# mickeyjoe666/PHFPFAC

Hardware: AMD Instinct MI355X
Metric: input GB/s scanned (higher is better)
Workload: dtype u8

## Files before the change

### phfpfac_amd/csrc/pfac_hip.hip

```cpp
#include <hip/hip_runtime.h>
#include <hip/hip_ext.h>

#include <stdint.h>
#include <stdio.h>
#include <stdlib.h>
#include <string.h>

#include <algorithm>
#include <chrono>
#include <mutex>
#include <type_traits>
#include <string>
#include <vector>

#include "pfac.h"
#include "pfac_fold.h"

namespace {

constexpr int WAVE = 64;
constexpr int SUB = WAVE * 16;
constexpr int SUBS = 4;
constexpr int WTILE = SUB * SUBS;
constexpr int MSUBS = 2;
// ... 749 lines not shown
    auto log_put = [&](bool f, unsigned word) {
        const unsigned long long b = __builtin_amdgcn_ballot_w64(f);
        if (b) {
            if (f) stg[(lc + lane_rank(b)) & (STG - 1u)] = word;
            lc += (unsigned)__popcll(b);
        }
    };
    auto log_flush = [&](bool all) {
        if (lc - fl >= (unsigned)WAVE || (all && lc != fl)) {
            wave_lds_sync();
            while (lc - fl >= (unsigned)WAVE) {
                __builtin_amdgcn_raw_buffer_store_b32(stg[(fl + (unsigned)lane) & (STG - 1u)], lrs, (int)((fl + (unsigned)lane) << 2), 0, 0);
                fl += WAVE;
            }
            if (all && fl + (unsigned)lane < lc)
                __builtin_amdgcn_raw_buffer_store_b32(stg[(fl + (unsigned)lane) & (STG - 1u)], lrs, (int)((fl + (unsigned)lane) << 2), 0, 0);
        }
    };
    auto slot = [&](int i) -> int4 {
        return *reinterpret_cast<const int4 *>(reinterpret_cast<const unsigned char *>(a.T4) + ((unsigned)i << 4));
    };
    auto slot_of = [&](int rnv, unsigned st, unsigned byte) -> int {
        return W8 ? rnv + (int)byte : rnv + (int)(((st & ((1u << sub) - 1u)) << 8) | byte);
    };
    const bool edge = own_end < (unsigned)WTILE || lim < (unsigned)WTILE + 3u;
    const unsigned n2 = (unsigned)a.d1_n2;
    auto front = [&](auto edge_c) {
        constexpr bool EDGE = decltype(edge_c)::value;
        unsigned p[D2_FB], win[D2_FB], rt[D2_FB], col[D2_FB];
        int nx[D2_FB];
        int2 e2[D2_FB];
#pragma unroll
        for (int u = 0; u < D2_FB; u++) {
            p[u] = P0 + (unsigned)(u * WAVE + lane);
            const unsigned lo = t32[p[u] >> 2], hi = t32[(p[u] >> 2) + 1];
            win[u] = __builtin_amdgcn_alignbyte(hi, lo, p[u] & 3u);
        }
#pragma unroll
        for (int u = 0; u < D2_FB; u++) {
            rt[u] = t0[win[u] & 0xFFu];
            col[u] = d1.colmap[(win[u] >> 8) & 0xFFu];
        }
#pragma unroll
        for (int u = 0; u < D2_FB; u++) {
            if (EDGE && p[u] >= own_end) rt[u] = no_root;
            nx[u] = d1.rows[(rt[u] >> 16) + col[u]];
        }
#pragma unroll
        for (int u = 0; u < D2_FB; u++) {
            if (EDGE && p[u] + 1u >= lim) nx[u] = -1;
            const unsigned ri = (unsigned)(nx[u] >> D1_STATE_BITS);
            e2[u] = d1.r2[ri < n2 ? ri : n2];
        }
#pragma unroll
        for (int u = 0; u < D2_FB; u++) {
            const unsigned s1 = rt[u] & 0xFFFFu, s2 = (unsigned)nx[u] & ((1u << D1_STATE_BITS) - 1u);
            const bool fin1 = s1 != 0xFFFFu, fin2 = s2 < nfin;
            const unsigned b2 = (win[u] >> 16) & 0xFFu;
#ifdef PFAC_ABL_D2NOWALK
            const bool more = false && b2;
#else
            const bool more = (((unsigned)e2[u].y >> (b2 & 31u)) & 1u) != 0u && (!EDGE || p[u] + 2u < lim);
#endif
            log_put(fin1, p[u] | (s1 << 16));
            log_put(fin2, p[u] | (fin1 ? 1u << 12 : 0u) | ((unsigned)nx[u] << 16));
            const unsigned long long mb = __builtin_amdgcn_ballot_w64(more);
            if (mb) {
                const unsigned n12 = (fin1 ? 1u : 0u) + (fin2 ? 1u : 0u);
                if (more) ring[(head + fcount + lane_rank(mb)) & (unsigned)(D2_RING - 1)] =
                    make_uint2(p[u] | ((unsigned)nx[u] << 12), (unsigned)slot_of(e2[u].x, s2, b2) | (n12 << 28));
                fcount += (unsigned)__popcll(mb);
            }
        }
        P0 += D2_FB * WAVE;
    };
#ifdef PFAC_TRACE_BUILD
    unsigned long long tq_front = 0, tq_iter = 0, tq_n = 0;
    const unsigned long long tq_t0 = __builtin_amdgcn_s_memrealtime();
#endif
    for (;;) {
        unsigned long long dm[NS];
        unsigned nd = 0;
#pragma unroll
        for (int w = 0; w < NS; w++) { dm[w] = __builtin_amdgcn_ballot_w64(!alive[w]); nd += (unsigned)__popcll(dm[w]); }
#ifdef PFAC_TRACE_BUILD
        const unsigned long long tq_a = __builtin_amdgcn_s_memrealtime();
#endif
        while (fcount < nd && P0 < own_end && fcount <= (unsigned)(D2_RING - D2_FB * WAVE)) {
            if (edge) front(std::true_type{}); else front(std::false_type{});
            log_flush(false);
        }
#ifdef PFAC_TRACE_BUILD
        tq_front += __builtin_amdgcn_s_memrealtime() - tq_a;
        tq_n++;
#endif
        if (nd == (unsigned)(NS * WAVE) && fcount == 0u) break;
        wave_lds_sync();
#pragma unroll
        for (int w = 0; w < NS; w++) {
            if (fcount && dm[w]) {
                const unsigned free_n = (unsigned)__popcll(dm[w]);
                const unsigned take = free_n < fcount ? free_n : fcount;
                const unsigned rk = lane_rank(dm[w]);
                if (!alive[w] && rk < take) {
                    const uint2 e = ring[(head + rk) & (unsigned)(D2_RING - 1)];
                    pos[w] = e.x & 0xFFFu;
                    s[w] = (int)(e.x >> 12);
                    idx[w] = (int)(e.y & 0x0FFFFFFFu);
                    jn[w] = e.y >> 28;
                    pn[w] = pos[w] + 2u;
                    alive[w] = true;
                }
                head += take;
                fcount -= take;
            }
        }
        int4 e4[NS];
        unsigned nb[NS];
#pragma unroll
        for (int w = 0; w < NS; w++) {
            e4[w] = make_int4(-1, -1, 0, 0);
            if (alive[w]) e4[w] = slot(idx[w]);
        }
#pragma unroll
        for (int w = 0; w < NS; w++) nb[w] = tile[alive[w] ? pn[w] + 1u : 0u];
#pragma unroll
        for (int w = 0; w < NS; w++) {
            const bool ok = alive[w] && e4[w].x == (W8 ? s[w] : (s[w] >> sub));
            const int sn = e4[w].y;
            const bool fin = ok && (unsigned)sn < nfin;
            log_put(fin, pos[w] | ((jn[w] & 15u) << 12) | ((unsigned)sn << 16));
            jn[w] += fin ? 1u : 0u;
            jmax |= jn[w];
            pn[w] += 1u;
            alive[w] = ok && pn[w] < lim && (((unsigned)e4[w].w >> (nb[w] & 31u)) & 1u) != 0u;
            s[w] = sn;
            idx[w] = slot_of(e4[w].z, (unsigned)sn, nb[w]);
        }
        log_flush(false);
    }
    log_flush(true);
#ifdef PFAC_TRACE_BUILD
    if (a.dbg && blockIdx.x < 8 && lane == 0 && (threadIdx.x >> 6) == 0) {
        unsigned long long *acc = a.dbg + (size_t)blockIdx.x * 64 * 32 + 10;
        const unsigned long long tq_all = __builtin_amdgcn_s_memrealtime() - tq_t0;
        acc[0] += tq_front; acc[1] += tq_n; acc[2] += tq_all; acc[3] += 1; acc[4] += lc;
    }
    (void)tq_iter;
#endif
    if (__any(jmax > 15u) || lc > logcap) return ~0u;
    return lc;
}

__device__ __forceinline__ void dense2_scatter(const ScanArgs &a, unsigned char *aux, const unsigned *logg, unsigned cnt,
                                               unsigned long long base, int lane) {
    unsigned *cntw = reinterpret_cast<unsigned *>(aux + D2_CNT_OFF);
    unsigned *pref2 = reinterpret_cast<unsigned *>(aux + D2_PREF_OFF);
    const unsigned short *pref = reinterpret_cast<const unsigned short *>(aux + D2_PREF_OFF);
    auto nibsum = [](unsigned x) -> unsigned { return (((x & 0x0F0F0F0Fu) + ((x >> 4) & 0x0F0F0F0Fu)) * 0x01010101u) >> 24; };
    constexpr int UN = 4;
    constexpr int ER = 32;
    const u32x4 zero4 = {0u, 0u, 0u, 0u};
    reinterpret_cast<u32x4 *>(cntw)[lane] = zero4;
    reinterpret_cast<u32x4 *>(cntw)[lane + WAVE] = zero4;
    wave_lds_sync();
    const unsigned long long room = base < a.out_cap ? a.out_cap - base : 0ull;
    const __amdgpu_buffer_rsrc_t ors = __builtin_amdgcn_make_buffer_rsrc(static_cast<unsigned *>(a.out) + base, 0,
                                                                         (int)((room < (unsigned long long)cnt ? (unsigned)room : cnt) * 4u), 0x00020000);
    auto count_one = [&](unsigned e) { atomicAdd(&cntw[(e & 0xFFFu) >> 3], 1u << ((e & 7u) * 4u)); };
    auto prefix = [&]() {
        wave_lds_sync();
        const u32x4 x0 = reinterpret_cast<const u32x4 *>(cntw)[2 * lane], x1 = reinterpret_cast<const u32x4 *>(cntw)[2 * lane + 1];
        unsigned sm[8];
#pragma unroll
        for (int k = 0; k < 4; k++) { sm[k] = nibsum(x0[k]); sm[4 + k] = nibsum(x1[k]); }
        unsigned tot = 0;
#pragma unroll
        for (int k = 0; k < 8; k++) tot += sm[k];
        unsigned run = wave_incl_scan(tot) - tot;
        u32x4 pw;
#pragma unroll
        for (int k = 0; k < 4; k++) {
            const unsigned lo = run; run += sm[2 * k];
            const unsigned hi = run; run += sm[2 * k + 1];
            pw[k] = lo | (hi << 16);
        }
        reinterpret_cast<u32x4 *>(pref2)[lane] = pw;
        wave_lds_sync();
    };
    auto place_one = [&](unsigned e) {
        const unsigned p = e & 0xFFFu, j = (e >> 12) & 15u, st = e >> 16;
        const unsigned x = cntw[p >> 3];
        const unsigned dest = (unsigned)pref[p >> 3] + nibsum(x & ((1u << ((p & 7u) * 4u)) - 1u)) + j;
        __builtin_amdgcn_raw_buffer_store_b32(p | (st << 12), ors, (int)(dest << 2), 0, 0);
    };
    if (cnt <= (unsigned)(ER * WAVE)) {
        const __amdgpu_buffer_rsrc_t lrs = __builtin_amdgcn_make_buffer_rsrc(const_cast<unsigned *>(logg), 0, (int)(cnt * 4u), 0x00020000);
        unsigned e[ER];
#pragma unroll
        for (int g = 0; g < ER / UN; g++) {
            if ((unsigned)(g * UN * WAVE) < cnt) {
#pragma unroll
                for (int u = 0; u < UN; u++)
                    e[g * UN + u] = __builtin_amdgcn_raw_buffer_load_b32(lrs, lane * 4, (g * UN + u) * WAVE * 4, 0);
            }
        }
#pragma unroll
        for (int g = 0; g < ER / UN; g++) {
            if ((unsigned)(g * UN * WAVE) < cnt) {
#pragma unroll
                for (int u = 0; u < UN; u++)
                    if ((unsigned)((g * UN + u) * WAVE + lane) < cnt) count_one(e[g * UN + u]);
            }
        }
        prefix();
#ifdef PFAC_ABL_D2NOSCATTER
        cnt = 0;
#endif
#pragma unroll
        for (int g = 0; g < ER / UN; g++) {
            if ((unsigned)(g * UN * WAVE) < cnt) {
#pragma unroll
                for (int u = 0; u < UN; u++)
                    if ((unsigned)((g * UN + u) * WAVE + lane) < cnt) place_one(e[g * UN + u]);
            }
        }
        return;
    }
    for (unsigned i0 = 0; i0 < cnt; i0 += UN * WAVE) {
        unsigned e[UN];
#pragma unroll
        for (int u = 0; u < UN; u++) {
            const unsigned i = i0 + (unsigned)(u * WAVE + lane);
            e[u] = i < cnt ? logg[i] : 0u;
        }
#pragma unroll
        for (int u = 0; u < UN; u++)
            if (i0 + (unsigned)(u * WAVE + lane) < cnt) count_one(e[u]);
    }
    prefix();
#ifdef PFAC_ABL_D2NOSCATTER
    cnt = 0;
#endif
    for (unsigned i0 = 0; i0 < cnt; i0 += UN * WAVE) {
        unsigned e[UN];
#pragma unroll
        for (int u = 0; u < UN; u++) {
            const unsigned i = i0 + (unsigned)(u * WAVE + lane);
            e[u] = i < cnt ? logg[i] : 0u;
        }
#pragma unroll
        for (int u = 0; u < UN; u++)
            if (i0 + (unsigned)(u * WAVE + lane) < cnt) place_one(e[u]);
    }
}

template <int ROOT>
__device__ __forceinline__ unsigned root_mask(const u32x4 w, const unsigned char *ftab, unsigned root_x4) {
    if (ROOT == 1) {
        unsigned nm[4];
#pragma unroll
        for (int i = 0; i < 4; i++) {
            const unsigned x = w[i] ^ root_x4;
            nm[i] = (((x & 0x7F7F7F7Fu) + 0x7F7F7F7Fu) | x) & 0x80808080u;
        }
        unsigned lo = __builtin_amdgcn_udot4(nm[0], 0x08040201u, 0u, false);
        lo = __builtin_amdgcn_udot4(nm[1], 0x80402010u, lo, false);
        unsigned hi = __builtin_amdgcn_udot4(nm[2], 0x08040201u, 0u, false);
        hi = __builtin_amdgcn_udot4(nm[3], 0x80402010u, hi, false);
        return ~((lo >> 7) | (hi << 1)) & 0xFFFFu;
    } else {
        const unsigned char *t8 = ftab;
        unsigned p = 0;
#pragma unroll
        for (int g = 0; g < 4; g++) {
            const unsigned d = w[g];
            const unsigned v = (unsigned)t8[d & 0xFFu] | (unsigned)t8[256 + ((d >> 8) & 0xFFu)] |
                               (unsigned)t8[512 + ((d >> 16) & 0xFFu)] | (unsigned)t8[768 + (d >> 24)];
            p |= v << (8 * g);
        }
        unsigned x = p & 0x0F0F0F0Fu, y = (p >> 4) & 0x0F0F0F0Fu;
        x = (x | (x >> 4)) & 0x00FF00FFu; y = (y | (y >> 4)) & 0x00FF00FFu;
        x = (x | (x >> 8)) & 0xFFFFu; y = (y | (y >> 8)) & 0xFFFFu;
        return x | (y << 16);
    }
}

__device__ __forceinline__ unsigned eq_mask32(const u32x4 lo16, const u32x4 hi16, unsigned x4) {
    return root_mask<1>(lo16, nullptr, x4) | (root_mask<1>(hi16, nullptr, x4) << 16);
}

#ifdef PFAC_TRACE_BUILD
#define PFAC_STAMP(cond, slot) do { if (cond) tr[slot] = __builtin_amdgcn_s_memrealtime(); } while (0)
#else
#define PFAC_STAMP(cond, slot) do { } while (0)
#endif

#ifndef PFAC_SPARSE_FUSED_NW
#define PFAC_SPARSE_FUSED_NW 2
#endif
constexpr int MAX_WAVES_NW4 = 10;

template <bool TLDS, bool W8, int ROOT, bool FUSED, int NW, int NB, bool FOLD>
__device__ __forceinline__ void scan_body(const ScanArgs &a, unsigned char *smem, const ErrCh &err) {
    unsigned *hdr = reinterpret_cast<unsigned *>(smem + SH_HDR);
    int *s0 = reinterpret_cast<int *>(smem + SH_S0);
    unsigned char *ftab = smem + SH_FTAB;
    unsigned char *finl = smem + SH_FIN;
    const int tid = threadIdx.x;
    const int lane = tid & (WAVE - 1);
    const int wave = __builtin_amdgcn_readfirstlane(tid >> 6);
    const int nc = (int)(blockDim.x >> 6) - 1;

    for (unsigned i = blockIdx.x * blockDim.x + tid; i < a.zero_vec; i += gridDim.x * blockDim.x)
        a.zero_next[i] = make_uint4(0u, 0u, 0u, 0u);
    for (int i = tid; i < H_WORDS; i += blockDim.x) hdr[i] = 0;
    for (int i = tid; i < 256; i += blockDim.x) {
        const int v = a.s0[i];
        const bool sec2 = a.sec2[i] != 0;
        s0[i] = v;
        finl[i] = (unsigned)v < (unsigned)a.num_final ? (unsigned char)1 : (unsigned char)0;
#pragma unroll
        for (int k = 0; k < 4; k++)
            ftab[k * 256 + i] = (unsigned char)((v >= 0 ? 1u << k : 0u) | (sec2 ? 1u << (k + 4) : 0u));
    }
    unsigned char *d1idx_l = smem + SH_D1IDX;
    int *d1_l = reinterpret_cast<int *>(smem + SH_D1);
    unsigned char *colmap_l = smem + SH_COLMAP;
    if (a.d1_rows > 0) {
        for (int i = tid; i < 256; i += blockDim.x) { d1idx_l[i] = a.d1idx[i]; colmap_l[i] = a.d1_colmap[i]; }
        for (int i = tid; i < a.d1_rows * a.d1_stride; i += blockDim.x) {
            const int row = i / a.d1_stride, c = i - row * a.d1_stride;
            d1_l[i] = c < a.d1_ncols ? a.d1[row * 256 + a.d1_colbyte[c]] : -1;
        }
    } else {
        for (int i = tid; i < 256; i += blockDim.x) { d1idx_l[i] = 0; colmap_l[i] = 0; }
    }
    if (a.d1_rows > 0)
        for (int i = tid; i < a.d1_stride; i += blockDim.x) d1_l[a.d1_rows * a.d1_stride + i] = -1;
    const unsigned *t0_l = reinterpret_cast<const unsigned *>(smem + a.sh_t0);
    if (FUSED && NW == 4 && a.sh_t0)
        for (int i = tid; i < 256; i += blockDim.x) {
            const int v = a.s0[i];
            reinterpret_cast<unsigned *>(smem + a.sh_t0)[i] = v >= 0 ? (((unsigned)v < (unsigned)a.num_final ? (unsigned)v : 0xFFFFu) | ((unsigned)(a.d1idx[i] * a.d1_stride) << 16))
                                                                     : (0xFFFFu | ((unsigned)(a.d1_rows * a.d1_stride) << 16));
        }
    int2 *d1r2_l = reinterpret_cast<int2 *>(smem + SH_D1 + a.d1_lds_bytes);
    if (FUSED && a.d1_n2 > 0)
        for (int i = tid; i <= a.d1_n2; i += blockDim.x) {
            const int2 e = i < a.d1_n2 ? a.d1r2[i] : make_int2(-a.rn_bias, 0);
            d1r2_l[i] = make_int2(e.x + a.rn_bias, e.y);
        }
    int *s0r_l = reinterpret_cast<int *>(smem + SH_D1);
    const bool have_s0r = FUSED && a.d1_rows == 0;
    if (have_s0r)
        for (int i = tid; i < 256; i += blockDim.x) {
            const int v = a.s0[i];
            s0r_l[i] = v >= 0 ? a.r[v >> (a.wbit - 8)] + a.rn_bias : 0;
        }
    const Dense1 d1 = {colmap_l, d1idx_l, d1_l, a.d1_rows > 0, (FUSED && a.d1_n2 > 0) ? d1r2_l : nullptr, have_s0r ? s0r_l : nullptr};
    const int sh_tab = SH_D1 + a.d1_lds_bytes;
    const int *R = a.r;
    const int2 *T = a.T;
    if (TLDS) {
        int *lr = reinterpret_cast<int *>(smem + sh_tab);
        int2 *lt = reinterpret_cast<int2 *>(smem + sh_tab + ((a.r_words * 4 + 15) & ~15));
        for (int i = tid; i < a.r_words; i += blockDim.x) lr[i] = a.r[i];
        for (int i = tid; i < a.t_entries; i += blockDim.x) lt[i] = a.T[i];
        R = lr;
        T = lt;
    }
    const unsigned char *bm2l = smem + a.sh_bm2;
    if (a.l2f_mode == 2) {
        const unsigned *src = reinterpret_cast<const unsigned *>(a.bm2 + (ROOT == 1 ? (a.root_byte & 0xFFu) * 32u : 0u));
        unsigned *dst = reinterpret_cast<unsigned *>(smem + a.sh_bm2);
        for (int i = tid; i < a.bm2_rows * 8; i += blockDim.x) dst[i] = src[i];
    }
    __syncthreads();
#ifdef PFAC_TRACE_BUILD
    if (a.dbg && blockIdx.x < 8 && threadIdx.x == 0) a.dbg[((size_t)blockIdx.x * 64 + 1) * 32 + 15] = __builtin_amdgcn_s_memrealtime();
#endif

#ifdef PFAC_ABL_NOCOORD
    if (wave == nc) return;
#endif
    if (wave == nc) {
        __builtin_amdgcn_s_setprio(3);
#ifdef PFAC_ABL_STATIC
        unsigned abl_seq = 0;
        auto ticket = [&]() -> unsigned { return (abl_seq++) * gridDim.x + blockIdx.x; };
#else
        auto ticket = [&]() -> unsigned {
            unsigned g = 0;
            if (lane == 0) g = atomicAdd(&a.ctl[(blockIdx.x % a.ticket_ways) * 64u], 1u) * a.ticket_ways + blockIdx.x % a.ticket_ways;
            return g;
        };
#endif
        auto publish_batch = [&](unsigned r, unsigned g_lane0) -> unsigned {
            if (lane == 0) {
                lds_store(&hdr[H_ARRIVED + (r & 7)], 0u);
                lds_store(&hdr[H_BATCH + (r & 7)], g_lane0);
                __builtin_amdgcn_fence(__ATOMIC_RELEASE, "workgroup");
                lds_store(&hdr[H_EPOCH + (r & 7)], r + 1);
            }
            return __builtin_amdgcn_readfirstlane(g_lane0);
        };
// ... 172 lines not shown
        if (more_far) issue_loads(t_far, w, hw);
        PFAC_STAMP(trace && r > 0, 10);
        auto emit_pending = [&](bool have, unsigned n_rec) {
            if (have && n_rec != 0) {
                unsigned long long base = 0;
                const bool okb = record_base(r - lag, base);
                PFAC_STAMP(trace, 9);
                if (okb) copy_out<!TLDS>(a, stage0 + (buf + 1u == nbuf ? 0u : buf + 1u) * a.stage_cap, n_rec, base, lane);
            }
        };
        if (NB == 3) emit_pending(pend_have[LAG_MAX - 1], pend_cnt[LAG_MAX - 1]);
        PFAC_STAMP(trace && r > 0, 11);

        unsigned keep[MSUBS] = {0u, 0u}, deep[MSUBS] = {0u, 0u};
        unsigned *stage = stage0 + buf * a.stage_cap;
        unsigned d2cnt = ~0u;
        if (NW == 4 && FUSED) {
            if (d2) {
                const unsigned long long own = a.n_owned - tile_base;
                d2cnt = dense2_tile<W8>(a, tile, t0_l, d1, aux, d2log, lane, lim, own < (unsigned long long)WTILE ? (unsigned)own : (unsigned)WTILE);
            }
        }
        const bool d2done = d2cnt != ~0u;
        PFAC_STAMP(trace && r > 0 && d2, 12);
        if (!d2done) {
#pragma unroll
        for (int j = 0; j < MSUBS; j++) {
            const unsigned off = j * MSUB + lane * MLANE;
            const u32x4 lo16 = *reinterpret_cast<const u32x4 *>(tile + off);
            const u32x4 hi16 = *reinterpret_cast<const u32x4 *>(tile + off + 16);
#ifdef PFAC_ABL_NOROOT
            const unsigned rlo = (lo16[0] == 0x12345678u), rhi = (hi16[0] == 0x12345678u);
#else
            const unsigned rlo = root_mask<ROOT>(lo16, ftab, a.root_byte), rhi = root_mask<ROOT>(hi16, ftab, a.root_byte);
#endif
            const unsigned raw = (rlo & 0xFFFFu) | (rhi << 16);
#ifdef PFAC_TRACE_BUILD
            asm volatile("" :: "v"(raw));
            PFAC_STAMP(trace && r > 0, j == 0 ? 12 : 14);
#endif
            unsigned m1 = raw;
            if (tile_base + WTILE > a.n_owned) {
                const unsigned long long g = tile_base + off;
                if (g + MLANE > a.n_owned) m1 = g >= a.n_owned ? 0u : (m1 & ((1u << (unsigned)(a.n_owned - g)) - 1u));
            }
            if (a.l2f_mode == 0) {
                keep[j] = m1;
                deep[j] = m1;
            } else if (ROOT == 1 && a.l2f_mode == 1) {
                unsigned nextc = 0;
                if (a.n_child > 0) {
                    const unsigned nx = *reinterpret_cast<const unsigned *>(tile + off + 32);
                    unsigned ec = a.child0 == a.root_byte ? raw : eq_mask32(lo16, hi16, a.child0);
                    unsigned e32 = ((nx ^ a.child0) & 0xFFu) == 0u ? 1u : 0u;
                    if (a.n_child > 1) {
                        ec |= a.child1 == a.root_byte ? raw : eq_mask32(lo16, hi16, a.child1);
                        e32 |= ((nx ^ a.child1) & 0xFFu) == 0u ? 1u : 0u;
                    }
                    nextc = (ec >> 1) | (e32 << 31);
                }
                deep[j] = m1 & nextc;
                keep[j] = root_final ? m1 : deep[j];
            } else {
                unsigned dm = 0, fm = 0;
                const unsigned *t32 = reinterpret_cast<const unsigned *>(tile);
                unsigned cand = m1;
                if (ROOT != 1 && a.sec_filter) {
                    const unsigned nx = *reinterpret_cast<const unsigned *>(tile + off + 32);
                    const unsigned s32 = ((unsigned)ftab[nx & 0xFFu] >> 4) & 1u;
                    cand = m1 & ((((rlo >> 16) | (rhi & 0xFFFF0000u)) >> 1) | (s32 << 31));
                }
#ifdef PFAC_ABL_NOCLASS
                cand = 0;
#endif
                if (ROOT != 1 && a.l2f_mode == 3) {
                    dm = cand;
                    cand = 0;
                }
                for (unsigned mm = cand; mm;) {
                    unsigned b[L2F_UNROLL], win[L2F_UNROLL], v[L2F_UNROLL], fin[L2F_UNROLL];
                    bool on[L2F_UNROLL];
#pragma unroll
                    for (int u = 0; u < L2F_UNROLL; u++) {
                        on[u] = mm != 0u;
                        b[u] = on[u] ? (unsigned)__ffs(mm) - 1u : 0u;
                        mm &= mm - 1u;
                        const unsigned p = off + b[u];
                        const unsigned lo = t32[p >> 2], hi = t32[(p >> 2) + 1];
                        win[u] = __builtin_amdgcn_alignbyte(hi, lo, p & 3u);
                    }
#pragma unroll
                    for (int u = 0; u < L2F_UNROLL; u++) {
                        const unsigned b0 = win[u] & 0xFFu, b1 = (win[u] >> 8) & 0xFFu;
                        v[u] = bm2l[(ROOT == 1 ? 0u : b0 * 32u) + (b1 >> 3)];
                        fin[u] = ROOT == 1 ? 0u : (unsigned)finl[b0];
                    }
#pragma unroll
                    for (int u = 0; u < L2F_UNROLL; u++) {
                        const unsigned b1 = (win[u] >> 8) & 0xFFu;
                        dm |= on[u] ? ((v[u] >> (b1 & 7u)) & 1u) << b[u] : 0u;
                        fm |= on[u] ? fin[u] << b[u] : 0u;
                    }
                }
                deep[j] = dm;
                keep[j] = dm | (ROOT == 1 ? (root_final ? m1 : 0u) : fm);
            }
#ifdef PFAC_TRACE_BUILD
            asm volatile("" :: "v"(keep[j]), "v"(deep[j]));
            PFAC_STAMP(trace && r > 0 && j == 0, 13);
#endif
        }
        }

#ifdef PFAC_ABL_NOKEEP
        asm volatile("" :: "v"(keep[0]), "v"(keep[1]), "v"(deep[0]), "v"(deep[1]));
        keep[0] = keep[1] = deep[0] = deep[1] = 0;
#endif
        PFAC_STAMP(trace, 6);
        const unsigned long long cnt = d2done ? (unsigned long long)d2cnt : !__any((keep[0] | keep[1]) != 0u) ? 0ull :
            tile_pass<W8, false, NW, FUSED, ROOT>(a, tile, s0, d1, R, T, q, stage, keep, deep, lane, lim, tile_base, 0);
        PFAC_STAMP(trace, 7);
#ifdef PFAC_TRACE_BUILD
        if (a.dbg && blockIdx.x < 8 && r < 64 && lane == 0) tr[16 + wave] = __builtin_amdgcn_s_memrealtime();
#endif
        const bool overflow = cnt > a.stage_cap;
        const bool now = overflow || nbuf == 1;
        unsigned arrival = 0;
#ifdef PFAC_ABL_NOCOORD
        if (false)
#endif
        if (lane == 0) {
            hdr[H_CNT + (r & 7) * 16 + wave] = (unsigned)cnt | ((now && cnt != 0) ? 0x80000000u : 0u);
            if (cnt > a.small_cap) {
                atomicAdd(&hdr[H_OVF2], 1u);
                if (cnt > a.sparse_cap) atomicAdd(&hdr[H_OVF], 1u);
            }
            __builtin_amdgcn_fence(__ATOMIC_RELEASE, "workgroup");
            arrival = atomicAdd(&hdr[H_ARRIVED + (r & 7)], 1u);
        }
        if (__builtin_amdgcn_readfirstlane(arrival) * 2u >= (unsigned)nc) __builtin_amdgcn_s_setprio(1);
        else __builtin_amdgcn_s_setprio(0);

        if (now && cnt != 0) {
            const unsigned long long take = a.rec_bytes == 2 ? (cnt + 7ull) & ~7ull : cnt;
            unsigned long long v = 0;
            if (lane == 0)
                v = __hip_atomic_fetch_add(reinterpret_cast<unsigned long long *>(a.ctl + CTL_CURSOR), take,
                                           __ATOMIC_RELAXED, __HIP_MEMORY_SCOPE_AGENT);
            const unsigned long long base = ((unsigned long long)__builtin_amdgcn_readfirstlane((unsigned)(v >> 32)) << 32) |
                                            __builtin_amdgcn_readfirstlane((unsigned)v);
            if (lane == 0) a.tile_index[t] = base | ((unsigned long long)cnt << TIX_CNT_SHIFT);
            PFAC_STAMP(trace && r > 0 && d2, 13);
            if (NW == 4 && FUSED && d2done) {
                dense2_scatter(a, aux, d2log, (unsigned)cnt, base, lane);
                PFAC_STAMP(trace && r > 0, 14);
            }
            else if (overflow)
                tile_pass<W8, true, NW, FUSED, ROOT>(a, tile, s0, d1, R, T, q, stage, keep, deep, lane, lim, tile_base, base);
            else
                copy_out<!TLDS>(a, stage, (unsigned)cnt, base, lane);
        }
        if (NB == 2) emit_pending(pend_have[0], pend_cnt[0]);
        PFAC_STAMP(trace, 8);
        if (NB == 3) { pend_have[LAG_MAX - 1] = pend_have[0]; pend_cnt[LAG_MAX - 1] = pend_cnt[0]; }
        pend_have[0] = !now; pend_cnt[0] = (unsigned)cnt;
        buf = buf + 1u >= nbuf ? 0u : buf + 1u;
        if (LOAD_DEPTH == 1) {
            if (!more_far) return false;
            t = t_far;
        } else {
            if (!have_n1) return false;
            t = t_n1;
            t_n1 = t_far;
            have_n1 = more_far;
        }
        r++;
        return true;
    };
    for (;;) {
        if (!round_body(wA, hA)) break;
        if (LOAD_DEPTH == 2 && !round_body(wB, hB)) break;
    }
#pragma unroll
    for (int k = LAG_MAX - 1; k >= 0; k--) {
        if ((unsigned)k < lag && pend_have[k] && pend_cnt[k] != 0) {
            unsigned long long base = 0;
            if (record_base(r - (unsigned)k, base))
                copy_out<!TLDS>(a, stage0 + ((buf + nbuf - 1u - (unsigned)k) % nbuf) * a.stage_cap, pend_cnt[k], base, lane);
        }
    }
}

template <bool TLDS, bool W8, int ROOT, bool FUSED, int NW, int NB = 2, bool FOLD = false>
__global__ __launch_bounds__(WAVE * MAX_WAVES_PER_BLOCK) void pfac_scan_kernel(ScanArgs a) {
    static_assert(NB == 2 || (NB == 3 && NW <= 3), "three staging buffers: the sparse-mode kernels (dense mode has one)");
    static_assert(!(TLDS && FUSED), "the fused table is for tables gathered through L2");
    static_assert(NW == (TLDS ? 1 : 2) || (FUSED && (NW == 3 || NW == 4)), "walks per lane: 1 (LDS tables), 2 (L2 tables), 3 (L2, fused), 4 (L2, fused, dense matches)");
    extern __shared__ __attribute__((aligned(16))) unsigned char smem[];
    const ErrCh err = {&a.ctl[CTL_ERR], a.spin_max};
#ifdef PFAC_TRACE_BUILD
    if (a.dbg && blockIdx.x < 8 && threadIdx.x == 0) a.dbg[((size_t)blockIdx.x * 64 + 0) * 32 + 15] = __builtin_amdgcn_s_memrealtime();
#endif
    if (blockIdx.x < T0_GROUPS && threadIdx.x == 0)
        (void)__hip_atomic_fetch_max(reinterpret_cast<unsigned long long *>(a.ctl + CTL_T0), ~__builtin_amdgcn_s_memrealtime(),
                                     __ATOMIC_RELAXED, __HIP_MEMORY_SCOPE_AGENT);
    scan_body<TLDS, W8, ROOT, FUSED, NW, NB, FOLD>(a, smem, err);
    unsigned *hdr = reinterpret_cast<unsigned *>(smem + SH_HDR);
    if ((threadIdx.x & (WAVE - 1)) == 0) {
        asm volatile("s_waitcnt vmcnt(0)" ::: "memory");
        const unsigned left = atomicAdd(&hdr[H_EXIT], 1u);
        if (left + 1 == (blockDim.x >> 6)) {
#ifdef PFAC_TRACE_BUILD
            if (a.dbg && blockIdx.x < 8) a.dbg[((size_t)blockIdx.x * 64 + 2) * 32 + 15] = __builtin_amdgcn_s_memrealtime();
#endif
            const unsigned done = __hip_atomic_fetch_add(&a.ctl[CTL_DONE], 1u, __ATOMIC_RELAXED, __HIP_MEMORY_SCOPE_AGENT);
            if (done + 1 == gridDim.x) {
                const unsigned long long tot = __hip_atomic_load(reinterpret_cast<unsigned long long *>(a.ctl + CTL_TOTAL), __ATOMIC_RELAXED, __HIP_MEMORY_SCOPE_AGENT);
                const unsigned long long cur = __hip_atomic_load(reinterpret_cast<unsigned long long *>(a.ctl + CTL_CURSOR), __ATOMIC_RELAXED, __HIP_MEMORY_SCOPE_AGENT);
                a.res[0] = (unsigned)tot; a.res[1] = (unsigned)(tot >> 32);
                a.res[2] = __hip_atomic_load(&a.ctl[CTL_ERR], __ATOMIC_RELAXED, __HIP_MEMORY_SCOPE_AGENT);
                a.res[3] = __hip_atomic_load(&a.ctl[CTL_OVF], __ATOMIC_RELAXED, __HIP_MEMORY_SCOPE_AGENT);
                a.res[4] = (unsigned)cur; a.res[5] = (unsigned)(cur >> 32);
                a.res[6] = __hip_atomic_load(&a.ctl[CTL_OVF2], __ATOMIC_RELAXED, __HIP_MEMORY_SCOPE_AGENT);
                const unsigned long long t0 = ~__hip_atomic_load(reinterpret_cast<unsigned long long *>(a.ctl + CTL_T0), __ATOMIC_RELAXED, __HIP_MEMORY_SCOPE_AGENT);
                const unsigned long long t1 = __builtin_amdgcn_s_memrealtime();
                a.res[RES_T0] = (unsigned)t0; a.res[RES_T0 + 1] = (unsigned)(t0 >> 32);
                a.res[RES_T1] = (unsigned)t1; a.res[RES_T1 + 1] = (unsigned)(t1 >> 32);
                __hip_atomic_store(&a.res[RES_DONE], 1u, __ATOMIC_RELEASE, __HIP_MEMORY_SCOPE_SYSTEM);
            }
        }
    }
}


__global__ void pfac_repack_kernel(const int *blob, int *s0, int *r, int2 *T, int *idmap, int max_row, int ht_size,
                                   int num_final, int state_num, int width, int *bad) {
    const int *b_s0 = blob + PFAC_BLOB_HEADER_WORDS;
    const int *b_r = b_s0 + 256;
    const int *b_HT = b_r + max_row;
    const int *b_val = b_HT + ht_size;
    const int *b_id = b_val + ht_size;
    const int stride = gridDim.x * blockDim.x;
    const int i0 = blockIdx.x * blockDim.x + threadIdx.x;
    bool ok = true;
    for (int i = i0; i < 256; i += stride) { s0[i] = b_s0[i]; ok = ok && b_s0[i] >= -1 && b_s0[i] < state_num; }
    for (int i = i0; i < max_row; i += stride) { r[i] = b_r[i]; ok = ok && b_r[i] > -width && b_r[i] < ht_size; }
    for (int i = i0; i < ht_size; i += stride) {
        T[i] = make_int2(b_HT[i], b_val[i]);
        ok = ok && (b_HT[i] < 0 || (b_val[i] >= -1 && b_val[i] < state_num));
    }
    for (int i = i0; i < num_final; i += stride) idmap[i] = b_id[i];
    if (!ok) *bad = 1;
}

__device__ __forceinline__ unsigned child_mask32(const int *r, const int2 *T, int wbit, int ht_size, int max_row, int state) {
    unsigned m = 0;
    if (state < 0) return 0u;
    for (int c = 0; c < 256; c++) {
        const int key = (state << 8) | c;
        const int row = key >> wbit;
        if (row >= max_row) continue;
        const int idx = r[row] + (key & ((1 << wbit) - 1));
        if ((unsigned)idx < (unsigned)ht_size) {
            const int2 e = T[idx];
            if (e.x == row && e.y >= 0) m |= 1u << (c & 31);
        }
    }
    return m;
}

__global__ void pfac_fuse_kernel(const int2 *T, const int *r, int wbit, int ht_size, int max_row, int4 *T4, int lo, int hi) {
    const int stride = gridDim.x * blockDim.x;
    for (int i = lo + blockIdx.x * blockDim.x + threadIdx.x; i < hi; i += stride) {
        const int2 e = (i >= 0 && i < ht_size) ? T[i] : make_int2(-1, -1);
        int rn = -1;
        bool have = false;
        if (e.y >= 0) {
            const int row = e.y >> (wbit - 8);
            if (row < max_row) { rn = r[row]; have = true; }
        }
        T4[i] = make_int4(e.x, e.y, have ? rn - lo : 0, e.x >= 0 ? (int)child_mask32(r, T, wbit, ht_size, max_row, e.y) : 0);
    }
}

__global__ void pfac_build_d1_kernel(const int *d1state, const int *r, const int2 *T, int wbit, int ht_size, int *d1) {
    const int st = d1state[blockIdx.x];
    const int c = threadIdx.x;
    const int key = (st << 8) | c;
    const int row = key >> wbit;
    const int idx = r[row] + (key & ((1 << wbit) - 1));
    int nx = -1;
    if ((unsigned)idx < (unsigned)ht_size) {
        const int2 e = T[idx];
        if (e.x == row) nx = e.y;
    }
    d1[blockIdx.x * 256 + c] = nx;
}

__global__ void pfac_pack_d1_kernel(int *d1, int n_entries, const int *r, const int2 *T, int wbit, int ht_size, int max_row, int2 *r2, int *counter) {
    const int i = blockIdx.x * blockDim.x + threadIdx.x;
    if (i >= n_entries) return;
    const int nx = d1[i];
    if (nx < 0) return;
    const int k = atomicAdd(counter, 1);
    const int row = nx >> (wbit - 8);
    r2[k] = make_int2(row < max_row ? r[row] : -1, (int)child_mask32(r, T, wbit, ht_size, max_row, nx));
    d1[i] = nx | (k << D1_STATE_BITS);
// ... 5121 lines not shown
```

Before: 5375.

## Stage dense2 scatter output in LDS windows and write coalesced vector stores

Instead of scattering each match record directly to global memory with per-lane buffer stores at arbitrary destinations, records are first placed into an LDS window (reusing the tile buffer) and then copied out with aligned 16-byte, optionally nontemporal, stores. Large logs are processed in multiple window passes that reread the log each time. The intent is to replace uncoalesced global scatter writes with coalesced ones. The cost is extra LDS traffic, wave syncs, and repeated log reads for logs bigger than one window.

```diff
diff --git a/phfpfac_amd/csrc/pfac_hip.hip b/phfpfac_amd/csrc/pfac_hip.hip
--- a/phfpfac_amd/csrc/pfac_hip.hip
+++ b/phfpfac_amd/csrc/pfac_hip.hip
@@ -925,8 +925,19 @@
     return lc;
 }
 
-__device__ __forceinline__ void dense2_scatter(const ScanArgs &a, unsigned char *aux, const unsigned *logg, unsigned cnt,
-                                               unsigned long long base, int lane) {
+#ifndef PFAC_D2_REC_AUX
+#define PFAC_D2_REC_AUX 1
+#endif
+#ifndef PFAC_D2_LOG_AUX
+#define PFAC_D2_LOG_AUX 0
+#endif
+constexpr bool D2_REC_NT = PFAC_D2_REC_AUX != 0;
+constexpr int D2_LOG_AUX = PFAC_D2_LOG_AUX;
+constexpr unsigned D2_WIN = (unsigned)(WTILE + D2_CNT_OFF) / 4u;
+static_assert(D2_WIN % 4u == 0u && D2_WIN >= 4u * WAVE, "windows begin on 16-byte boundaries of the record array");
+__device__ __forceinline__ void dense2_scatter(const ScanArgs &a, unsigned char *tile, unsigned char *aux, const unsigned *logg,
+                                               unsigned cnt, unsigned long long base, int lane) {
+    unsigned *win = reinterpret_cast<unsigned *>(tile);
     unsigned *cntw = reinterpret_cast<unsigned *>(aux + D2_CNT_OFF);
     unsigned *pref2 = reinterpret_cast<unsigned *>(aux + D2_PREF_OFF);
     const unsigned short *pref = reinterpret_cast<const unsigned short *>(aux + D2_PREF_OFF);
@@ -937,9 +948,9 @@
     reinterpret_cast<u32x4 *>(cntw)[lane] = zero4;
     reinterpret_cast<u32x4 *>(cntw)[lane + WAVE] = zero4;
     wave_lds_sync();
-    const unsigned long long room = base < a.out_cap ? a.out_cap - base : 0ull;
-    const __amdgpu_buffer_rsrc_t ors = __builtin_amdgcn_make_buffer_rsrc(static_cast<unsigned *>(a.out) + base, 0,
-                                                                         (int)((room < (unsigned long long)cnt ? (unsigned)room : cnt) * 4u), 0x00020000);
+    const unsigned sh = (unsigned)base & 3u, vend = sh + cnt;
+    unsigned *o = static_cast<unsigned *>(a.out) + (base - sh);
+    const bool checked = base + cnt > a.out_cap;
     auto count_one = [&](unsigned e) { atomicAdd(&cntw[(e & 0xFFFu) >> 3], 1u << ((e & 7u) * 4u)); };
     auto prefix = [&]() {
         wave_lds_sync();
@@ -961,11 +972,33 @@
         reinterpret_cast<u32x4 *>(pref2)[lane] = pw;
         wave_lds_sync();
     };
-    auto place_one = [&](unsigned e) {
+    auto place_one = [&](unsigned e, bool have, unsigned w0) -> bool {
         const unsigned p = e & 0xFFFu, j = (e >> 12) & 15u, st = e >> 16;
         const unsigned x = cntw[p >> 3];
-        const unsigned dest = (unsigned)pref[p >> 3] + nibsum(x & ((1u << ((p & 7u) * 4u)) - 1u)) + j;
-        __builtin_amdgcn_raw_buffer_store_b32(p | (st << 12), ors, (int)(dest << 2), 0, 0);
+        const unsigned v = sh + (unsigned)pref[p >> 3] + nibsum(x & ((1u << ((p & 7u) * 4u)) - 1u)) + j;
+        const unsigned rel = v - w0;
+        if (have && rel < D2_WIN) win[rel] = p | (st << 12);
+        return have && v >= w0 + D2_WIN;
+    };
+    auto window_out = [&](unsigned w0) {
+        wave_lds_sync();
+        const unsigned lo = w0 > sh ? w0 : sh, hi = w0 + D2_WIN < vend ? w0 + D2_WIN : vend;
+        if (checked) {
+            for (unsigned v = lo + (unsigned)lane; v < hi; v += WAVE)
+                if (base - sh + v < a.out_cap) o[v] = win[v - w0];
+        } else {
+            unsigned b0 = (lo + 3u) & ~3u;
+            b0 = b0 < hi ? b0 : hi;
+            const unsigned b1 = b0 + ((hi - b0) & ~3u);
+            if (lo + (unsigned)lane < b0) o[lo + lane] = win[lo + lane - w0];
+            for (unsigned v = b0 + 4u * (unsigned)lane; v < b1; v += 4u * WAVE) {
+                const u32x4 r4 = *reinterpret_cast<const u32x4 *>(win + (v - w0));
+                if (D2_REC_NT) __builtin_nontemporal_store(r4, reinterpret_cast<u32x4 *>(o + v));
+                else *reinterpret_cast<u32x4 *>(o + v) = r4;
+            }
+            if (b1 + (unsigned)lane < hi) o[b1 + lane] = win[b1 + lane - w0];
+        }
+        wave_lds_sync();
     };
     if (cnt <= (unsigned)(ER * WAVE)) {
         const __amdgpu_buffer_rsrc_t lrs = __builtin_amdgcn_make_buffer_rsrc(const_cast<unsigned *>(logg), 0, (int)(cnt * 4u), 0x00020000);
@@ -975,7 +1008,7 @@
             if ((unsigned)(g * UN * WAVE) < cnt) {
 #pragma unroll
                 for (int u = 0; u < UN; u++)
-                    e[g * UN + u] = __builtin_amdgcn_raw_buffer_load_b32(lrs, lane * 4, (g * UN + u) * WAVE * 4, 0);
+                    e[g * UN + u] = __builtin_amdgcn_raw_buffer_load_b32(lrs, lane * 4, (g * UN + u) * WAVE * 4, D2_LOG_AUX);
             }
         }
 #pragma unroll
@@ -988,15 +1021,33 @@
         }
         prefix();
 #ifdef PFAC_ABL_D2NOSCATTER
-        cnt = 0;
+        return;
 #endif
+        static_assert((unsigned)(ER * WAVE) + 3u <= 2u * D2_WIN, "a log that fits the registers fits two windows");
+        unsigned later = 0;
 #pragma unroll
         for (int g = 0; g < ER / UN; g++) {
             if ((unsigned)(g * UN * WAVE) < cnt) {
+                bool l = false;
 #pragma unroll
                 for (int u = 0; u < UN; u++)
-                    if ((unsigned)((g * UN + u) * WAVE + lane) < cnt) place_one(e[g * UN + u]);
+                    l |= place_one(e[g * UN + u], (unsigned)((g * UN + u) * WAVE + lane) < cnt, 0u);
+                if (__any(l)) later |= 1u << g;
             }
+        }
+        window_out(0u);
+        if (later) {
+#pragma unroll
+            for (int g = 0; g < ER / UN; g++) {
+                if ((later >> g) & 1u) {
+#pragma unroll
+                    for (int u = 0; u < UN; u++) {
+                        asm volatile("" : "+v"(e[g * UN + u]));
+                        place_one(e[g * UN + u], (unsigned)((g * UN + u) * WAVE + lane) < cnt, D2_WIN);
+                    }
+                }
+            }
+            window_out(D2_WIN);
         }
         return;
     }
@@ -1013,18 +1064,20 @@
     }
     prefix();
 #ifdef PFAC_ABL_D2NOSCATTER
-    cnt = 0;
+    return;
 #endif
-    for (unsigned i0 = 0; i0 < cnt; i0 += UN * WAVE) {
-        unsigned e[UN];
-#pragma unroll
-        for (int u = 0; u < UN; u++) {
-            const unsigned i = i0 + (unsigned)(u * WAVE + lane);
-            e[u] = i < cnt ? logg[i] : 0u;
-        }
-#pragma unroll
-        for (int u = 0; u < UN; u++)
-            if (i0 + (unsigned)(u * WAVE + lane) < cnt) place_one(e[u]);
+    for (unsigned w0 = 0; w0 < vend; w0 += D2_WIN) {
+        for (unsigned i0 = 0; i0 < cnt; i0 += UN * WAVE) {
+            unsigned e[UN];
+#pragma unroll
+            for (int u = 0; u < UN; u++) {
+                const unsigned i = i0 + (unsigned)(u * WAVE + lane);
+                e[u] = i < cnt ? logg[i] : 0u;
+            }
+#pragma unroll
+            for (int u = 0; u < UN; u++) place_one(e[u], i0 + (unsigned)(u * WAVE + lane) < cnt, w0);
+        }
+        window_out(w0);
     }
 }
 
@@ -1503,7 +1556,7 @@
             if (lane == 0) a.tile_index[t] = base | ((unsigned long long)cnt << TIX_CNT_SHIFT);
             PFAC_STAMP(trace && r > 0 && d2, 13);
             if (NW == 4 && FUSED && d2done) {
-                dense2_scatter(a, aux, d2log, (unsigned)cnt, base, lane);
+                dense2_scatter(a, tile, aux, d2log, (unsigned)cnt, base, lane);
                 PFAC_STAMP(trace && r > 0, 14);
             }
             else if (overflow)
```

Result: no change. 5377 (median of 3 runs) (+0.0%).
